# HaoZhongkai/DPOT

Measured on AMD Instinct MI355X. Metric: PDE samples/sec (128^2 x10 -> 1 rollout step), DPOT-Tiny train step, higher is better.
Workload: dtype f32

## Files before the change

### dpot_amd/_lib.py

```python
from __future__ import annotations

import ctypes as C
import os
import threading

HERE = os.path.dirname(os.path.abspath(__file__))
LIB_PATH = os.environ.get("DPOT_HIP_LIB") or os.path.join(HERE, "lib", "libdpot_hip.so")

c_fp = C.c_void_p
c_i = C.c_int
c_i64 = C.c_int64
c_f = C.c_float
c_d = C.c_double


class GemmDesc(C.Structure):
    _fields_ = [
        ("A", c_fp), ("B", c_fp), ("C", c_fp),
        ("M", C.c_int32), ("N", C.c_int32), ("K", C.c_int32),
        ("batch", C.c_int32),
        ("transA", C.c_int32), ("transB", C.c_int32),
        ("lda", C.c_int32), ("ldb", C.c_int32), ("ldc", C.c_int32),
        ("strideA", c_i64), ("strideB", c_i64), ("strideC", c_i64),
        ("bias", c_fp), ("strideBias", c_i64),
# ... 157 lines not shown
    "dpot_mlp_wgrad2": (c_i, [c_fp] * 4 + [c_i] * 3 + [c_fp] * 5 + [c_i, c_fp]),
    "dpot_afno_wgrad2_splitk": (c_i, [c_i] * 3),
    "dpot_afno_wgrad2_ws_elems": (c_i64, [c_i] * 3),
    "dpot_afno_wgrad2": (c_i, [c_fp] * 4 + [c_i] * 4 + [c_fp] * 5 + [c_i, c_fp]),
    "dpot_block_finalize": (c_i, [c_fp, c_i, c_i, c_i] + [c_fp] * 4 + [c_fp, c_i, c_i, c_i] + [c_fp] * 4 + [c_fp] * 3
                            + [c_i, c_i, c_i] + [c_fp] * 4 + [c_i, c_fp]),
    "dpot_bf16_pack_both_supported": (c_i, [c_i, c_i]),
    "dpot_bf16_pack_both": (c_i, [c_fp, c_i, c_i, c_i, c_fp, c_fp, c_fp, c_fp]),
    "dpot_bf16_pack_both_norm": (c_i, [c_fp, c_i, c_i, c_i, c_fp, c_fp, c_fp, c_fp, c_i, c_i, c_fp, c_fp, c_fp]),
    "dpot_embed_supported": (c_i, [c_i] * 5),
    "dpot_embed_wfrag_elems": (c_i, []),
    "dpot_embed_pack_w0": (c_i, [c_fp, c_i, c_fp, c_fp]),
    "dpot_embed_fwd": (c_i, [c_fp] * 5 + [c_i] * 6 + [c_fp]),
    "dpot_embed_wgrad_ws_elems": (c_i, [c_i] * 3),
    "dpot_embed_wgrad": (c_i, [c_fp] * 4 + [c_i] * 7 + [c_fp]),
    "dpot_gemm_panel_supported": (c_i, [c_i, c_i, c_i]),
    "dpot_gemm_panel": (c_i, [c_fp, c_i, c_fp, c_fp, c_fp, c_i, c_fp, c_i, c_fp, c_i, c_fp, c_i] + [c_i] * 5 + [c_fp]),
}

_lib = None
_lock = threading.Lock()


class DpotHipError(RuntimeError):
    pass


def lib_path() -> str:
    return LIB_PATH

# ... 26 lines not shown
```

### dpot_amd/build.py

```python
from __future__ import annotations

import os
import shutil
import subprocess
import sys
from concurrent.futures import ThreadPoolExecutor

HERE = os.path.dirname(os.path.abspath(__file__))
CSRC = os.path.join(HERE, "csrc")
LIBDIR = os.path.join(HERE, "lib")
LIB = os.path.join(LIBDIR, "libdpot_hip.so")
SOURCES = ["core.hip", "gemm.hip", "gemm_panel.hip", "gemm_tn.hip", "gemm_bf16p.hip", "afno_mlp.hip", "afno_mlp6.hip", "afno_fused.hip", "dft.hip", "norm.hip", "gn_dft.hip", "misc.hip", "loss_opt.hip", "metrics.hip", "tail.hip", "data.hip", "embed.hip", "resize.hip", "evalmetrics.hip"]
FLAGS = ["--offload-arch=gfx950", "-O3", "-std=c++17", "-fPIC", "-Wall", "-Wno-unused-function",
         "-Wno-pass-failed"]
EXTRA_FLAGS = {"afno_mlp6.hip": ["-fno-slp-vectorize"]}


def _hipcc() -> str:
    for cand in (os.environ.get("HIPCC"), shutil.which("hipcc"), "/opt/rocm/bin/hipcc"):
        if cand and os.path.exists(cand):
            return cand
    raise RuntimeError("hipcc not found (need ROCm >= 7.0 to build the gfx950 kernels)")


def _stale(target: str, deps) -> bool:
    if not os.path.exists(target):
        return True
    t = os.path.getmtime(target)
    return any(os.path.getmtime(d) > t for d in deps)


def build(force: bool = False, verbose: bool = True) -> str:
    hipcc = _hipcc()
    os.makedirs(LIBDIR, exist_ok=True)
    hdrs = [os.path.join(CSRC, "common.h"), os.path.join(CSRC, "dft_fast.h"), os.path.join(CSRC, "gemm_split.h"), os.path.join(CSRC, "gemm_epi.h"), os.path.join(CSRC, "gemm_bf16p_common.h"), os.path.join(os.path.dirname(HERE), "include", "dpot_hip.h")]
    objs, jobs = [], []
    for src in SOURCES:
        s = os.path.join(CSRC, src)
        o = os.path.join(LIBDIR, src.replace(".hip", ".o"))
        objs.append(o)
        if force or _stale(o, [s] + hdrs):
            jobs.append([hipcc] + FLAGS + EXTRA_FLAGS.get(src, []) + ["-c", s, "-o", o])

    def run(cmd):
        if verbose:
            print("[dpot_amd.build]", " ".join(cmd), flush=True)
        r = subprocess.run(cmd, capture_output=True, text=True)
        if r.returncode != 0:
            raise RuntimeError(f"hipcc failed:\n{' '.join(cmd)}\n{r.stdout}\n{r.stderr}")
        return r
# ... 12 lines not shown
```

### dpot_amd/csrc/embed.hip

```cpp
#include "common.h"

namespace dpot {

typedef float f32x4 __attribute__((ext_vector_type(4)));

constexpr int EM_P = 8;
constexpr int EM_C = 4;
constexpr int EM_NP = 4;
constexpr int EM_CT = 3;
constexpr int EM_LW = 2;
constexpr int EM_TMAX = 10;
constexpr int EM_KD = EM_C * EM_P * EM_P;
constexpr int EM_WFL = EM_P * 2 * EM_CT * 256;
constexpr int EM_GFL = EM_P * EM_NP * EM_P * EM_TMAX * EM_C;

struct EmbedArgs {
  const float* x;
  const float* wf;
  const float* bt;
  const float* dh;
  float* hpre;
  float* hh;
  float* part;
  int X, Y, T, h, w, hidp, act, ngroups, wq;
};

__device__ __forceinline__ void em_glds16(const float* g, float* l) {
  __builtin_amdgcn_global_load_lds((const __attribute__((address_space(1))) void*)g,
// ... 230 lines not shown
  for (int s = s0; s < s1; ++s) v += part[((long long)s * 48 + n) * EM_KD + k];
  red[sl][o] = v;
  __syncthreads();
  if (sl == 0 && ok) {
    float t = 0.f;
#pragma unroll
    for (int q = 0; q < 16; ++q) t += red[q][o];
    dw0[(long long)n * ldw + k] = t;
  }
}

__global__ __launch_bounds__(256) void embed_pack_w0_kernel(const float* __restrict__ w0, int hid, int K0,
                                                            float* __restrict__ wf) {
  const int idx = blockIdx.x * 256 + threadIdx.x;
  if (idx >= EM_WFL) return;
  const int jj = idx & 3, lane = (idx >> 2) & 63, blk = idx >> 8;
  const int ct = blk % EM_CT, ij = blk / EM_CT;
  const int jq = ij & 1, i = ij >> 1;
  const int n = ct * 16 + (lane & 15), c = lane >> 4;
  wf[idx] = n < hid ? w0[(long long)n * K0 + c * 64 + i * 8 + 4 * jq + jj] : 0.f;
}

}

using namespace dpot;

static int embed_grid(int ngroups) {
  int g = ngroups < 256 ? ngroups : 256;
  return g < 1 ? 1 : g;
}

extern "C" int dpot_embed_supported(int C, int P, int T, int hid, int w) {
  return C == EM_C && P == EM_P && T >= 1 && T <= EM_TMAX && hid >= 1 && hid <= 16 * EM_CT && w % EM_NP == 0;
}

// ... 62 lines not shown
```

### dpot_amd/functional.py

```python
from __future__ import annotations

import os
from collections import OrderedDict
from typing import Optional

import torch

from . import ops
from .ops import EPI_ACT, EPI_DACT

Tensor = torch.Tensor


def _pad4(n: int) -> int:
    return (n + 3) // 4 * 4


class _Sink:
    __slots__ = ("fp", "i")

    def __init__(self, param: Optional[Tensor], needed: bool):
        s = getattr(param, "_dpot_grad_slot", None) if (needed and param is not None) else None
        self.fp, self.i = s if s is not None else (None, -1)
        if self.fp is not None:
# ... 62 lines not shown

def embed_derived(pos, w0, b0, w2, b2, taw, tagamma, tt, T: int, grid=None, layouts=None):
    hid, E = w0.shape[0], w2.shape[0]
    K0 = w0[0].numel()
    hidp = _pad4(hid)
    tok = pos.shape[2] * pos.shape[3]
    dev = pos.device
    if layouts is not None:
        w0p, b0p, w2p, posb = layouts[0].view(hidp, K0), layouts[1].view(hidp), layouts[2].view(E, hidp), layouts[3].view(tok, E)
    else:
        w0p = ops.copy2d_pad(w0, hid, K0, hidp, K0)
        b0p = ops.copy2d_pad(b0, 1, hid, 1, hidp).view(hidp)
        w2p = ops.copy2d_pad(w2, E, hid, E, hidp)
        posT = ops.transpose2d(pos, 1, E, tok).view(tok, E)
        posb = ops.bias_add(posT, b2)
    ws = ops.timeagg_scale_w(taw, tagamma, tt) if tagamma is not None else taw
    V = torch.empty(T * hidp, E, dtype=torch.float32, device=dev)
    ops.gemm(w2p, ws, V, hidp, E, E, transA=True, lda=hidp, ldb=E, ldc=E, batch=T, strideA=0, strideB=E * E,
             strideC=hidp * E)
    wsum = ops.colsum(ws, T, E * E).view(E, E)
    cc = torch.empty(tok, E, dtype=torch.float32, device=dev)
    ops.gemm(posb, wsum, cc, tok, E, E, lda=E, ldb=E, ldc=E)
    wfrag = bt = None
    if grid is not None:
        kg = grid.shape[1]
        wfrag = ops.embed_pack_w0(w0)
        bt = torch.empty(grid.shape[0], hidp, dtype=torch.float32, device=dev)
        ops.gemm(grid, w0p[:, K0 - kg:], bt, grid.shape[0], hidp, kg, transB=True, lda=kg, ldb=K0, ldc=hidp, bias=b0p)
    return w0p, b0p, w2p, posb, ws, V, wsum, cc, wfrag, bt, grid

# ... 38 lines not shown
        _check_epoch(ctx, "EmbedFn")
        A0, Hpre, Hh, w0p, w2p, ws, V, wsum, posb, taw, tagamma, tt, grid = ctx.saved_tensors
        B, X, Y, T, Cc, P, h, w, hid, hidp, E, K0, act = ctx.dims
        s_pos, s_w0, s_b0, s_w2, s_b2, s_taw, s_gamma = ctx.sinks
        tok = h * w
        M, M0 = B * tok, B * tok * T
        dev = dY.device
        dY = dY.contiguous().view(M, E)
        dHpre = torch.empty(M0, hidp, dtype=torch.float32, device=dev)
        ops.gemm(dY, V, dHpre, M, T * hidp, E, transB=True, lda=E, ldb=E, ldc=T * hidp, act=act, mode=EPI_DACT,
                 aux=Hpre, ldaux=T * hidp)
        dV = torch.empty(T * hidp, E, dtype=torch.float32, device=dev)
        ops.gemm(Hh, dY, dV, T * hidp, E, M, transA=True, lda=T * hidp, ldb=E, ldc=E,
                 splitk=ops.auto_splitk(T * hidp, E, M, tn=True))
        dc = ops.group_rowsum(dY, B, tok, 1, E)
        dwsum = torch.empty(E, E, dtype=torch.float32, device=dev)
        ops.gemm(posb, dc, dwsum, E, E, tok, transA=True, lda=E, ldb=E, ldc=E, splitk=ops.auto_splitk(E, E, tok, tn=True))
        dposb = torch.empty(tok, E, dtype=torch.float32, device=dev)
        ops.gemm(dc, wsum, dposb, tok, E, E, transB=True, lda=E, ldb=E, ldc=E)
        dpos = s_pos.done(ops.transpose2d(dposb, 1, tok, E, out=s_pos.out()).view(1, E, h, w))
        db2 = s_b2.done(ops.colsum(dposb, tok, E, out=s_b2.out()))
        dw2_t = torch.empty(T, E, hidp, dtype=torch.float32, device=dev)
        ops.gemm(ws, dV, dw2_t, E, hidp, E, transB=True, lda=E, ldb=E, ldc=hidp, batch=T, strideA=E * E,
                 strideB=hidp * E, strideC=E * hidp)
        dw2p = ops.colsum(dw2_t, T, E * hidp).view(E, hidp)
        dw2 = s_w2.done(ops.copy2d_pad(dw2p, E, hidp, E, hid, out=s_w2.out()).view(E, hid, 1, 1))
        dws = s_taw.out() if tagamma is None else None
        dws = ops._out(dws, (T, E, E), dev)
        ops.gemm(w2p, dV, dws, E, E, hidp, lda=hidp, ldb=E, ldc=E, batch=T, strideA=0, strideB=hidp * E,
                 strideC=E * E, res=dwsum, ldres=E, strideRes=0)
        if tagamma is not None:
            dtaw, dgamma = ops.timeagg_scale_w_bwd(dws, taw, tagamma, tt, out_dw=s_taw.out(),
                                                   out_dgamma=s_gamma.out())
            dtaw, dgamma = s_taw.done(dtaw), s_gamma.done(dgamma)
        else:
            dtaw, dgamma = s_taw.done(dws), None
        if ctx.implicit:
            db0 = s_b0.done(ops.colsum(dHpre, M0, hid, ld=hidp, out=s_b0.out()))
            dw0 = ops._out(s_w0.out(), (hid, K0), dev)
            ops.embed_wgrad(A0, dHpre, dw0, hid)
            dHs = ops.group_rowsum(dHpre, B, tok * T, 1, hidp)
            kg = grid.shape[1]
            ops.gemm(dHs, grid, dw0[:, K0 - kg:], hid, kg, tok * T, transA=True, lda=hidp, ldb=kg, ldc=K0)
            dw0 = s_w0.done(dw0.view(hid, Cc + 3, P, P))
        elif hid == hidp:
            dw0p, db0 = ops.linear_bwd_wb(dHpre, A0, None, s_b0.out())
            db0 = s_b0.done(db0)
        else:
            db0 = s_b0.done(ops.colsum(dHpre, M0, hid, ld=hidp, out=s_b0.out()))
            dw0p = ops.linear_bwd_weight(dHpre, A0)
        if not ctx.implicit:
            dw0 = s_w0.done(ops.copy2d_pad(dw0p, hidp, K0, hid, K0, out=s_w0.out()).view(hid, Cc + 3, P, P))
        dx = None
        if ctx.needs_input_grad[0]:
            dA0 = ops.linear_bwd_data(dHpre, w0p)
            dx = ops.unpatchify(dA0, B, X, Y, T, Cc, P)
        return dx, dpos, dw0, db0, dw2, db2, dtaw, dgamma, None, None, None, None, None, None, None

# ... 651 lines not shown
```

### dpot_amd/ops.py

```python
from __future__ import annotations

import ctypes as C
import contextlib
import functools
import threading
import os
from typing import Optional, Tuple

import torch

from . import _lib
from ._lib import GemmDesc, check

Tensor = torch.Tensor

ACT_IDS = {None: 0, "none": 0, "gelu": 1, "tanh": 2, "sigmoid": 3, "relu": 4, "leaky_relu": 5, "softplus": 6,
           "ELU": 7, "silu": 8}
EPI_LINEAR, EPI_ACT, EPI_DACT, EPI_AFNO_WGRAD = 0, 1, 2, 3
GEMM_F32, GEMM_BF16X6, GEMM_AUTO, GEMM_BF16 = 0, 1, 2, 3
_PRECISIONS = {"f32": GEMM_F32, "bf16x6": GEMM_BF16X6, "auto": GEMM_AUTO, "bf16": GEMM_BF16}
_gemm_precision = _PRECISIONS[os.environ.get("DPOT_GEMM_PRECISION", "f32")]


def set_gemm_precision(name: str) -> None:
# ... 91 lines not shown
TUNE_KEYS = {
    "mixer": (3, "AFNO mixer MLP: 3 = three-product fused kernel (afno_mlp3), 4 = four-product fused kernel (afno_mlp2), "
                 "0 = two generic GEMM launches"),
    "afno_layer": (-1, "one-launch AFNO layer forward (afno_fused_fwd): -1 = where it measured faster (>= 80 % full last "
                       "round of (sample, block) workgroups), 0 = never, 1 = wherever supported"),
    "gn_fuse": (1, "0 = GroupNorm as its own kernels: not fused with the mixer's DFTs, never applied on the load of its consumer"),
    "panel": (1, "0 = generic GEMM kernels instead of the pre-packed-weight panel GEMM, the token-contraction weight-gradient "
                 "kernels (gemm_tn) and their two-layer launches"),
    "wgrad_gauss": (1, "0 = four-product AFNO weight gradients instead of the three-product forms"),
    "bf16p_bd": (1, "0 = the LDS-DMA bf16 GEMM kernels of rounds 2-3 for every launch instead of the B-direct kernels"),
    "bf16p_shape": (1, "0 = none of the bf16 GEMM shape heuristics: 128 x 256 tiles only, column-major tile order, eight waves, "
                       "un-paired weight gradients"),
    "packs": (1, "0 = bf16 packs by separate pack passes only: none from the one-launch AFNO layer, the GroupNorm backward or Adam"),
    "pack_both": (1, "0 = bf16 channel MLP without the pack-both path (one pack pass per operand form, fp32 pre-activation saved)"),
    "fused_small": (1, "0 = separate small launches: per-block reduce launches, eight layout launches, torch ops for the cls head"),
    "embed_implicit": (1, "0 = explicit patch matrix + GEMM instead of the implicit-GEMM patch embedding"),
    "mixer6": (1, "bf16x6 mixer kernel afno_mlp6 under gemm_precision 'auto' / 'bf16x6': 1 = where it measured faster (96 channels "
                  "per block: DPOT-L), 2 = wherever supported (also 128), 0 = never (the fp32 matrix-core kernels)"),
}


def _parse_tune():
    out = {}
    for kv in os.environ.get("DPOT_TUNE", "").split(","):
        kv = kv.strip()
        if not kv:
            continue
        k, _, v = kv.partition("=")
        if k not in TUNE_KEYS:
            raise ValueError(f"DPOT_TUNE: unknown key {k!r} (known: {', '.join(TUNE_KEYS)})")
        out[k] = int(v)
# ... 765 lines not shown
    M0 = B * (X // 8) * (Y // 8) * T
    hpre = torch.empty(M0, hidp, dtype=torch.float32, device=x.device)
    hh = torch.empty_like(hpre)
    check(_lib.load().dpot_embed_fwd(x.data_ptr(), wfrag.data_ptr(), btab.data_ptr(), hpre.data_ptr(), hh.data_ptr(),
                                     B, X, Y, T, hidp, act, _stream()), "embed_fwd")
    return hh, hpre


def embed_wgrad(x: Tensor, dhpre: Tensor, dw0: Tensor, hid: int) -> Tensor:
    lib = _lib.load()
    B, X, Y, T, _ = x.shape
    ws = torch.empty(lib.dpot_embed_wgrad_ws_elems(B, X, Y), dtype=torch.float32, device=x.device)
    check(lib.dpot_embed_wgrad(x.data_ptr(), dhpre.data_ptr(), ws.data_ptr(), dw0.data_ptr(), dw0.stride(0), hid, B, X,
                               Y, T, dhpre.shape[1], _stream()), "embed_wgrad")
    return dw0


def unpatchify(dA: Tensor, B: int, X: int, Y: int, T: int, Cc: int, P: int) -> Tensor:
    dx = torch.empty(B, X, Y, T, Cc, dtype=torch.float32, device=dA.device)
    check(_lib.load().dpot_unpatchify(dA.data_ptr(), dx.data_ptr(), B, X, Y, T, Cc, P, _stream()), "unpatchify")
    return dx


def pixel_shuffle(z: Tensor, B: int, h: int, w: int, P: int, Cc: int, inverse: bool = False) -> Tensor:
    out = torch.empty(B * h * w * P * P, Cc, dtype=torch.float32, device=z.device)
    if not inverse:
        out = out.view(B, h * P, w * P, Cc)
        check(_lib.load().dpot_pixel_shuffle(z.data_ptr(), out.data_ptr(), B, h, w, P, Cc, 0, _stream()),
              "pixel_shuffle")
    else:
# ... 729 lines not shown
```

### include/dpot_hip.h

```cpp
#ifndef DPOT_HIP_H
#define DPOT_HIP_H

#include <stdint.h>

#ifdef __cplusplus
extern "C" {
#endif

#define DPOT_OK 0
#define DPOT_EINVAL (-1)
#define DPOT_EUNSUP (-2)
#define DPOT_EHIP (-3)

typedef void* dpot_stream_t;

enum {
  DPOT_ACT_NONE = 0,
  DPOT_ACT_GELU = 1,
  DPOT_ACT_TANH = 2,
  DPOT_ACT_SIGMOID = 3,
  DPOT_ACT_RELU = 4,
  DPOT_ACT_LEAKY_RELU = 5,
  DPOT_ACT_SOFTPLUS = 6,
  DPOT_ACT_ELU = 7,
// ... 130 lines not shown
                        dpot_stream_t stream);

int dpot_patchify(const float* x, const float* gx, const float* gy, const float* gt, float* A, int B, int X,
                  int Y, int T, int C, int P, dpot_stream_t stream);
int dpot_unpatchify(const float* dA, float* dx, int B, int X, int Y, int T, int C, int P,
                    dpot_stream_t stream);

int dpot_embed_supported(int C, int P, int T, int hid, int w);
int dpot_embed_wfrag_elems(void);
int dpot_embed_pack_w0(const float* w0, int hid, float* wfrag, dpot_stream_t stream);
int dpot_embed_fwd(const float* x, const float* wfrag, const float* btab, float* hpre, float* hh, int B, int X, int Y,
                   int T, int hidp, int act, dpot_stream_t stream);
int dpot_embed_wgrad_ws_elems(int B, int X, int Y);
int dpot_embed_wgrad(const float* x, const float* dhpre, float* workspace, float* dw0, int ldw, int hid, int B, int X,
                     int Y, int T, int hidp, dpot_stream_t stream);
int dpot_pixel_shuffle(const float* z, float* out, int B, int h, int w, int P, int Cc, int inverse,
                       dpot_stream_t stream);
int dpot_copy2d_pad(const float* src, int sR, int sC, float* dst, int dR, int dC, dpot_stream_t stream);
int dpot_transpose2d(const float* src, float* dst, int nbatch, int R, int C, dpot_stream_t stream);
int dpot_colsum_parts(int M);
int dpot_colsum(const float* X, int M, int N, int ld, float* out, float* part, dpot_stream_t stream);
int dpot_colsum_scatter(const float* X, int M, int N, int ld, float* part, int nseg, const int* seg_start,
                        const int* seg_len, float* const* seg_dst, dpot_stream_t stream);
int dpot_group_rowsum(const float* X, float* out, int B, int R, int T, int N, dpot_stream_t stream);
int dpot_token_mean(const float* x, float* y, int B, int T, int E, dpot_stream_t stream);
int dpot_token_mean_bwd(const float* dy, const float* add, float* dx, int B, int T, int E,
                        dpot_stream_t stream);
int dpot_small_linear_supported(int M, int N, int K);
int dpot_small_linear(const float* x, int ldx, const float* W, int ldw, const float* bias, float* y, float* pre, int ldy,
                      int M, int N, int K, int act, dpot_stream_t stream);
// ... 177 lines not shown
```

Baseline: 10640.

## Fuse embed-fold weight-only algebra into multi-segment forward and backward kernels

Adds embed_fold kernels that compute the weight-only parts of the patch-embedding fold in a few segmented launches: the time-aggregation products V, the weight sum over T, the positional term, the grid bias table and the w0 fragment packing on the forward side, and dpos, db2, dw2, dtaw, dgamma and the grid part of dw0 on the backward side. These replace many separate generic GEMM, colsum and copy launches. The goal is to cut launch count and host overhead for small weight-only work on each train step. The cost is a large new code path with hand-written fp32 MFMA tiles and partial-sum workspaces that need their own reductions. It is gated by embed_implicit and E<=512.

After: 10630. Within noise of the previous version (-0.1%).

```diff
diff --git a/dpot_amd/_lib.py b/dpot_amd/_lib.py
--- a/dpot_amd/_lib.py
+++ b/dpot_amd/_lib.py
@@ -195,6 +195,10 @@
     "dpot_embed_fwd": (c_i, [c_fp] * 5 + [c_i] * 6 + [c_fp]),
     "dpot_embed_wgrad_ws_elems": (c_i, [c_i] * 3),
     "dpot_embed_wgrad": (c_i, [c_fp] * 4 + [c_i] * 7 + [c_fp]),
+    "dpot_embed_fold_supported": (c_i, [c_i] * 4),
+    "dpot_embed_fold_bwd_ws_elems": (c_i64, [c_i] * 5),
+    "dpot_embed_fold_fwd": (c_i, [c_fp] * 15 + [c_i] * 7 + [c_fp]),
+    "dpot_embed_fold_bwd": (c_i, [c_fp] * 16 + [c_i, c_fp] + [c_i] * 7 + [c_fp]),
     "dpot_gemm_panel_supported": (c_i, [c_i, c_i, c_i]),
     "dpot_gemm_panel": (c_i, [c_fp, c_i, c_fp, c_fp, c_fp, c_i, c_fp, c_i, c_fp, c_i, c_fp, c_i] + [c_i] * 5 + [c_fp]),
 }
diff --git a/dpot_amd/build.py b/dpot_amd/build.py
--- a/dpot_amd/build.py
+++ b/dpot_amd/build.py
@@ -10,7 +10,7 @@
 CSRC = os.path.join(HERE, "csrc")
 LIBDIR = os.path.join(HERE, "lib")
 LIB = os.path.join(LIBDIR, "libdpot_hip.so")
-SOURCES = ["core.hip", "gemm.hip", "gemm_panel.hip", "gemm_tn.hip", "gemm_bf16p.hip", "afno_mlp.hip", "afno_mlp6.hip", "afno_fused.hip", "dft.hip", "norm.hip", "gn_dft.hip", "misc.hip", "loss_opt.hip", "metrics.hip", "tail.hip", "data.hip", "embed.hip", "resize.hip", "evalmetrics.hip"]
+SOURCES = ["core.hip", "gemm.hip", "gemm_panel.hip", "gemm_tn.hip", "gemm_bf16p.hip", "afno_mlp.hip", "afno_mlp6.hip", "afno_fused.hip", "dft.hip", "norm.hip", "gn_dft.hip", "misc.hip", "loss_opt.hip", "metrics.hip", "tail.hip", "data.hip", "embed.hip", "embed_fold.hip", "resize.hip", "evalmetrics.hip"]
 FLAGS = ["--offload-arch=gfx950", "-O3", "-std=c++17", "-fPIC", "-Wall", "-Wno-unused-function",
          "-Wno-pass-failed"]
 EXTRA_FLAGS = {"afno_mlp6.hip": ["-fno-slp-vectorize"]}
@@ -33,7 +33,7 @@
 def build(force: bool = False, verbose: bool = True) -> str:
     hipcc = _hipcc()
     os.makedirs(LIBDIR, exist_ok=True)
-    hdrs = [os.path.join(CSRC, "common.h"), os.path.join(CSRC, "dft_fast.h"), os.path.join(CSRC, "gemm_split.h"), os.path.join(CSRC, "gemm_epi.h"), os.path.join(CSRC, "gemm_bf16p_common.h"), os.path.join(os.path.dirname(HERE), "include", "dpot_hip.h")]
+    hdrs = [os.path.join(CSRC, "common.h"), os.path.join(CSRC, "dft_fast.h"), os.path.join(CSRC, "gemm_split.h"), os.path.join(CSRC, "gemm_epi.h"), os.path.join(CSRC, "gemm_bf16p_common.h"), os.path.join(CSRC, "embed_pack.h"), os.path.join(os.path.dirname(HERE), "include", "dpot_hip.h")]
     objs, jobs = [], []
     for src in SOURCES:
         s = os.path.join(CSRC, src)
diff --git a/dpot_amd/csrc/embed.hip b/dpot_amd/csrc/embed.hip
--- a/dpot_amd/csrc/embed.hip
+++ b/dpot_amd/csrc/embed.hip
@@ -1,17 +1,12 @@
 #include "common.h"
+#include "embed_pack.h"
 
 namespace dpot {
 
 typedef float f32x4 __attribute__((ext_vector_type(4)));
 
-constexpr int EM_P = 8;
-constexpr int EM_C = 4;
-constexpr int EM_NP = 4;
-constexpr int EM_CT = 3;
 constexpr int EM_LW = 2;
 constexpr int EM_TMAX = 10;
-constexpr int EM_KD = EM_C * EM_P * EM_P;
-constexpr int EM_WFL = EM_P * 2 * EM_CT * 256;
 constexpr int EM_GFL = EM_P * EM_NP * EM_P * EM_TMAX * EM_C;
 
 struct EmbedArgs {
@@ -272,11 +267,7 @@
                                                             float* __restrict__ wf) {
   const int idx = blockIdx.x * 256 + threadIdx.x;
   if (idx >= EM_WFL) return;
-  const int jj = idx & 3, lane = (idx >> 2) & 63, blk = idx >> 8;
-  const int ct = blk % EM_CT, ij = blk / EM_CT;
-  const int jq = ij & 1, i = ij >> 1;
-  const int n = ct * 16 + (lane & 15), c = lane >> 4;
-  wf[idx] = n < hid ? w0[(long long)n * K0 + c * 64 + i * 8 + 4 * jq + jj] : 0.f;
+  wf[idx] = em_pack_w0_elem(w0, hid, K0, idx);
 }
 
 }
diff --git a/dpot_amd/csrc/embed_fold.hip b/dpot_amd/csrc/embed_fold.hip
--- /dev/null
+++ b/dpot_amd/csrc/embed_fold.hip
@@ -0,0 +1,440 @@
+#include "common.h"
+#include "embed_pack.h"
+
+namespace dpot {
+
+typedef float ef_f32x4 __attribute__((ext_vector_type(4)));
+
+constexpr int EF_KC = 32;
+constexpr int EF_LD = 65;
+constexpr int EF_EMAX = 2048;
+constexpr int EF_TMAX = 64;
+constexpr int EF_WR = 4;
+constexpr int EF_KS = 256;
+
+struct EfArgs {
+  const float *taw, *gamma, *tt, *w2p, *posb, *w0, *w0p, *b0p, *grid, *wsum_in, *dV, *dc, *dHs;
+  float *V, *wsum, *cc, *wfrag, *bt, *ws, *dpos, *db2, *dw2, *dtaw, *dgamma, *dw0;
+  float *k_dwsum, *k_db2, *k_dw2, *k_dw0, *k_dg;
+  int T, E, hidp, hid, tok, K0, kg, R, ldw0;
+  int e0, e1, e2, e3;
+  int nks, nrt, njt;
+};
+
+__device__ __forceinline__ float ef_cos(const EfArgs& a, int t, int i) {
+  return a.gamma ? cosf(a.tt[t] * a.gamma[i]) : 1.f;
+}
+
+template <int BM, int BN, bool AKF, bool BKF, class FA, class FB>
+__device__ __forceinline__ void ef_gemm(ef_f32x4 (&acc)[BM / 32][BN / 32], int K, FA fa, FB fb, float* As, float* Bs) {
+  constexpr int NA = BM * EF_KC / 256, NB = BN * EF_KC / 256, TM = BM / 32, TN = BN / 32;
+  const int tid = threadIdx.x, lane = tid & 63, wid = tid >> 6;
+  const int wm = (wid & 1) * (BM / 2), wn = (wid >> 1) * (BN / 2);
+  float ra[NA], rb[NB];
+#pragma unroll
+  for (int i = 0; i < TM; ++i)
+#pragma unroll
+    for (int j = 0; j < TN; ++j) acc[i][j] = ef_f32x4{0.f, 0.f, 0.f, 0.f};
+  auto gload = [&](int k0) {
+#pragma unroll
+    for (int r = 0; r < NA; ++r) {
+      const int idx = tid + 256 * r;
+      const int k = AKF ? idx % EF_KC : idx / BM, m = AKF ? idx / EF_KC : idx % BM;
+      ra[r] = k0 + k < K ? fa(m, k0 + k) : 0.f;
+    }
+#pragma unroll
+    for (int r = 0; r < NB; ++r) {
+      const int idx = tid + 256 * r;
+      const int k = BKF ? idx % EF_KC : idx / BN, n = BKF ? idx / EF_KC : idx % BN;
+      rb[r] = k0 + k < K ? fb(k0 + k, n) : 0.f;
+    }
+  };
+  gload(0);
+  for (int k0 = 0; k0 < K; k0 += EF_KC) {
+#pragma unroll
+    for (int r = 0; r < NA; ++r) {
+      const int idx = tid + 256 * r;
+      const int k = AKF ? idx % EF_KC : idx / BM, m = AKF ? idx / EF_KC : idx % BM;
+      As[k * EF_LD + m] = ra[r];
+    }
+#pragma unroll
+    for (int r = 0; r < NB; ++r) {
+      const int idx = tid + 256 * r;
+      const int k = BKF ? idx % EF_KC : idx / BN, n = BKF ? idx / EF_KC : idx % BN;
+      Bs[k * EF_LD + n] = rb[r];
+    }
+    __syncthreads();
+    if (k0 + EF_KC < K) gload(k0 + EF_KC);
+    const int kend = min(EF_KC, K - k0);
+    for (int kk = 0; kk < kend; kk += 4) {
+      const int kr = (kk + (lane >> 4)) * EF_LD + (lane & 15);
+      float af[TM], bf[TN];
+#pragma unroll
+      for (int i = 0; i < TM; ++i) af[i] = As[kr + wm + i * 16];
+#pragma unroll
+      for (int j = 0; j < TN; ++j) bf[j] = Bs[kr + wn + j * 16];
+#pragma unroll
+      for (int i = 0; i < TM; ++i)
+#pragma unroll
+        for (int j = 0; j < TN; ++j) acc[i][j] = __builtin_amdgcn_mfma_f32_16x16x4f32(af[i], bf[j], acc[i][j], 0, 0, 0);
+    }
+    __syncthreads();
+  }
+}
+
+template <int BM, int BN, class EPI>
+__device__ __forceinline__ void ef_epilogue(const ef_f32x4 (&acc)[BM / 32][BN / 32], EPI epi) {
+  const int lane = threadIdx.x & 63, wid = threadIdx.x >> 6;
+  const int wm = (wid & 1) * (BM / 2), wn = (wid >> 1) * (BN / 2);
+#pragma unroll
+  for (int i = 0; i < BM / 32; ++i)
+#pragma unroll
+    for (int j = 0; j < BN / 32; ++j)
+#pragma unroll
+      for (int r = 0; r < 4; ++r) epi(wm + i * 16 + 4 * (lane >> 4) + r, wn + j * 16 + (lane & 15), acc[i][j][r]);
+}
+
+template <int BM, int BN, class F>
+__device__ __forceinline__ float ef_rowsum(const ef_f32x4 (&acc)[BM / 32][BN / 32], F f, float* red) {
+  const int lane = threadIdx.x & 63, wid = threadIdx.x >> 6;
+  const int wm = (wid & 1) * (BM / 2), wn = (wid >> 1) * (BN / 2);
+#pragma unroll
+  for (int i = 0; i < BM / 32; ++i)
+#pragma unroll
+    for (int r = 0; r < 4; ++r) {
+      const int m = wm + i * 16 + 4 * (lane >> 4) + r;
+      float s = 0.f;
+#pragma unroll
+      for (int j = 0; j < BN / 32; ++j) s += f(m, wn + j * 16 + (lane & 15), acc[i][j][r]);
+#pragma unroll
+      for (int off = 8; off > 0; off >>= 1) s += __shfl_xor(s, off, 64);
+      if ((lane & 15) == 0) red[(wid >> 1) * BM + m] = s;
+    }
+  __syncthreads();
+  return threadIdx.x < BM ? red[threadIdx.x] + red[BM + threadIdx.x] : 0.f;
+}
+
+__global__ __launch_bounds__(256) void embed_fold_fwd_kernel(const EfArgs a) {
+  __shared__ float As[EF_KC * EF_LD], Bs[EF_KC * EF_LD], aux[EF_EMAX];
+  const int tid = threadIdx.x, E = a.E, hidp = a.hidp;
+  int b = blockIdx.x;
+  if (b < a.e0) {
+    const int nct = E / 32, t = b / nct, j0 = (b - t * nct) * 32;
+    for (int i = tid; i < E; i += 256) aux[i] = ef_cos(a, t, i);
+    __syncthreads();
+    const float* tw = a.taw + (long long)t * E * E;
+    ef_f32x4 acc[2][1];
+    ef_gemm<64, 32, false, false>(
+        acc, E, [&](int m, int k) { return m < hidp ? a.w2p[k * hidp + m] : 0.f; },
+        [&](int k, int n) { return tw[(long long)k * E + j0 + n] * aux[k]; }, As, Bs);
+    float* Vt = a.V + (long long)t * hidp * E;
+    ef_epilogue<64, 32>(acc, [&](int m, int n, float v) {
+      if (m < hidp) Vt[(long long)m * E + j0 + n] = v;
+    });
+    return;
+  }
+  b -= a.e0;
+  if (b < a.e1 - a.e0) {
+    const int i0 = b * EF_WR, T = a.T;
+    for (int q = tid; q < T * EF_WR; q += 256) aux[q] = ef_cos(a, q / EF_WR, min(i0 + q % EF_WR, E - 1));
+    __syncthreads();
+    for (int e = tid; e < EF_WR * E; e += 256) {
+      const int r = e / E, j = e - r * E, i = i0 + r;
+      if (i >= E) break;
+      float s = 0.f;
+      for (int t = 0; t < T; ++t) {
+        const long long o = ((long long)t * E + i) * E + j;
+        const float v = a.taw[o] * aux[t * EF_WR + r];
+        if (a.ws) a.ws[o] = v;
+        s += v;
+      }
+      a.wsum[(long long)i * E + j] = s;
+    }
+    return;
+  }
+  b -= a.e1 - a.e0;
+  if (b < a.e2 - a.e1) {
+    const int q0 = b * 64, kg = a.kg, R = a.R, K0 = a.K0;
+    ef_f32x4 acc[2][2];
+    ef_gemm<64, 64, true, true>(
+        acc, kg, [&](int m, int k) { return q0 + m < R ? a.grid[(long long)(q0 + m) * kg + k] : 0.f; },
+        [&](int k, int n) { return n < hidp ? a.w0p[(long long)n * K0 + (K0 - kg) + k] : 0.f; }, As, Bs);
+    ef_epilogue<64, 64>(acc, [&](int m, int n, float v) {
+      if (q0 + m < R && n < hidp) a.bt[(long long)(q0 + m) * hidp + n] = v + a.b0p[n];
+    });
+    return;
+  }
+  b -= a.e2 - a.e1;
+  const int idx = b * 256 + tid;
+  if (idx < EM_WFL) a.wfrag[idx] = em_pack_w0_elem(a.w0, a.hid, a.K0, idx);
+}
+
+template <int BT>
+__global__ __launch_bounds__(256) void embed_fold_cc_kernel(const EfArgs a) {
+  __shared__ float As[EF_KC * EF_LD], Bs[EF_KC * EF_LD];
+  const int E = a.E, tok = a.tok, nct = E / BT;
+  const int r0 = (blockIdx.x / nct) * BT, j0 = (blockIdx.x % nct) * BT;
+  ef_f32x4 acc[BT / 32][BT / 32];
+  ef_gemm<BT, BT, true, false>(
+      acc, E, [&](int m, int k) { return r0 + m < tok ? a.posb[(long long)(r0 + m) * E + k] : 0.f; },
+      [&](int k, int n) { return a.wsum[(long long)k * E + j0 + n]; }, As, Bs);
+  ef_epilogue<BT, BT>(acc, [&](int m, int n, float v) {
+    if (r0 + m < tok) a.cc[(long long)(r0 + m) * E + j0 + n] = v;
+  });
+}
+
+template <int BT>
+__global__ __launch_bounds__(256) void embed_fold_bwd1_kernel(const EfArgs a) {
+  __shared__ float As[EF_KC * EF_LD], Bs[EF_KC * EF_LD], aux[128];
+  const int tid = threadIdx.x, E = a.E, hidp = a.hidp, tok = a.tok;
+  int b = blockIdx.x;
+  if (b < a.e0) {
+    const int nrt = (tok + BT - 1) / BT, it = b / nrt, rt = b - it * nrt;
+    const int i0 = it * BT, r0 = rt * BT;
+    ef_f32x4 acc[BT / 32][BT / 32];
+    ef_gemm<BT, BT, true, true>(
+        acc, E, [&](int m, int k) { return a.wsum_in[(long long)(i0 + m) * E + k]; },
+        [&](int k, int n) { return r0 + n < tok ? a.dc[(long long)(r0 + n) * E + k] : 0.f; }, As, Bs);
+    ef_epilogue<BT, BT>(acc, [&](int m, int n, float v) {
+      if (r0 + n < tok) a.dpos[(long long)(i0 + m) * tok + r0 + n] = v;
+    });
+    const float s = ef_rowsum<BT, BT>(acc, [&](int, int n, float v) { return r0 + n < tok ? v : 0.f; }, aux);
+    if (tid < BT) a.k_db2[(long long)rt * E + i0 + tid] = s;
+    return;
+  }
+  b -= a.e0;
+  if (b < a.e1 - a.e0) {
+    const int nct = E / BT, i0 = (b / nct) * BT, j0 = (b % nct) * BT;
+    ef_f32x4 acc[BT / 32][BT / 32];
+    ef_gemm<BT, BT, false, false>(
+        acc, tok, [&](int m, int k) { return a.posb[(long long)k * E + i0 + m]; },
+        [&](int k, int n) { return a.dc[(long long)k * E + j0 + n]; }, As, Bs);
+    ef_epilogue<BT, BT>(acc, [&](int m, int n, float v) { a.k_dwsum[(long long)(i0 + m) * E + j0 + n] = v; });
+    return;
+  }
+  b -= a.e1 - a.e0;
+  if (b < a.e2 - a.e1) {
+    const int nit = E / 32, t = b / nit, i0 = (b - t * nit) * 32;
+    if (tid < 32) aux[tid] = ef_cos(a, t, i0 + tid);
+    __syncthreads();
+    const float* tw = a.taw + (long long)t * E * E;
+    const float* dVt = a.dV + (long long)t * hidp * E;
+    ef_f32x4 acc[1][2];
+    ef_gemm<32, 64, true, true>(
+        acc, E, [&](int m, int k) { return tw[(long long)(i0 + m) * E + k] * aux[m]; },
+        [&](int k, int n) { return n < hidp ? dVt[(long long)n * E + k] : 0.f; }, As, Bs);
+    float* part = a.k_dw2 + (long long)t * E * hidp;
+    ef_epilogue<32, 64>(acc, [&](int m, int n, float v) {
+      if (n < hidp) part[(long long)(i0 + m) * hidp + n] = v;
+    });
+    return;
+  }
+  b -= a.e2 - a.e1;
+  {
+    const int kg = a.kg, R = a.R, nkt = (kg + 31) / 32;
+    const int s = b / nkt, c0 = (b - s * nkt) * 32;
+    const int q0 = s * EF_KS, kl = min(EF_KS, R - q0);
+    ef_f32x4 acc[2][1];
+    ef_gemm<64, 32, false, false>(
+        acc, kl, [&](int m, int k) { return m < hidp ? a.dHs[(long long)(q0 + k) * hidp + m] : 0.f; },
+        [&](int k, int n) { return c0 + n < kg ? a.grid[(long long)(q0 + k) * kg + c0 + n] : 0.f; }, As, Bs);
+    float* part = a.k_dw0 + (long long)s * hidp * kg;
+    ef_epilogue<64, 32>(acc, [&](int m, int n, float v) {
+      if (m < hidp && c0 + n < kg) part[(long long)m * kg + c0 + n] = v;
+    });
+  }
+}
+
+__global__ __launch_bounds__(256) void embed_fold_bwd2_kernel(const EfArgs a) {
+  __shared__ float As[EF_KC * EF_LD], Bs[EF_KC * EF_LD], aux[128], red[128];
+  const int tid = threadIdx.x, E = a.E, hidp = a.hidp, T = a.T;
+  int b = blockIdx.x;
+  if (b < a.e0) {
+    const int nt = E / 64, t = b / (nt * nt), q = b - t * nt * nt, i0 = (q / nt) * 64, jt = q % nt, j0 = jt * 64;
+    if (tid < 64) {
+      float cs = 1.f, coef = 0.f;
+      if (a.gamma) {
+        const float tv = a.tt[t], arg = tv * a.gamma[i0 + tid];
+        cs = cosf(arg);
+        coef = -sinf(arg) * tv;
+      }
+      aux[tid] = cs;
+      aux[64 + tid] = coef;
+    }
+    __syncthreads();
+    const float* dVt = a.dV + (long long)t * hidp * E;
+    ef_f32x4 acc[2][2];
+    ef_gemm<64, 64, true, false>(
+        acc, hidp, [&](int m, int k) { return a.w2p[(long long)(i0 + m) * hidp + k]; },
+        [&](int k, int n) { return dVt[(long long)k * E + j0 + n]; }, As, Bs);
+    const long long base = (long long)t * E * E;
+#pragma unroll
+    for (int i = 0; i < 2; ++i)
+#pragma unroll
+      for (int j = 0; j < 2; ++j)
+#pragma unroll
+        for (int r = 0; r < 4; ++r) {
+          const int lane = tid & 63, wid = tid >> 6;
+          const int m = (wid & 1) * 32 + i * 16 + 4 * (lane >> 4) + r, n = (wid >> 1) * 32 + j * 16 + (lane & 15);
+          acc[i][j][r] += a.k_dwsum[(long long)(i0 + m) * E + j0 + n];
+        }
+    ef_epilogue<64, 64>(acc, [&](int m, int n, float v) {
+      a.dtaw[base + (long long)(i0 + m) * E + j0 + n] = v * aux[m];
+    });
+    if (a.gamma) {
+      const float s = ef_rowsum<64, 64>(
+          acc, [&](int m, int n, float v) { return v * a.taw[base + (long long)(i0 + m) * E + j0 + n]; }, red);
+      if (tid < 64) a.k_dg[((long long)t * a.njt + jt) * E + i0 + tid] = s * aux[64 + tid];
+    }
+    return;
+  }
+  b -= a.e0;
+  if (b < a.e1 - a.e0) {
+    const int i = b * 256 + tid;
+    if (i < E) {
+      float s = 0.f;
+      for (int p = 0; p < a.nrt; ++p) s += a.k_db2[(long long)p * E + i];
+      a.db2[i] = s;
+    }
+    return;
+  }
+  b -= a.e1 - a.e0;
+  if (b < a.e2 - a.e1) {
+    const int idx = b * 256 + tid, hid = a.hid;
+    if (idx < E * hid) {
+      const int i = idx / hid, h = idx - i * hid;
+      float s = 0.f;
+      for (int t = 0; t < T; ++t) s += a.k_dw2[((long long)t * E + i) * hidp + h];
+      a.dw2[idx] = s;
+    }
+    return;
+  }
+  b -= a.e2 - a.e1;
+  {
+    const int idx = b * 256 + tid, kg = a.kg, nks = a.nks;
+    if (idx < a.hid * kg) {
+      const int n = idx / kg, k = idx - n * kg;
+      float s = 0.f;
+      for (int p = 0; p < nks; ++p) s += a.k_dw0[((long long)p * hidp + n) * kg + k];
+      a.dw0[(long long)n * a.ldw0 + (a.K0 - kg) + k] = s;
+    }
+  }
+}
+
+__global__ __launch_bounds__(256) void embed_fold_dgamma_kernel(const float* __restrict__ part, int nparts, int E,
+                                                                float* __restrict__ dgamma) {
+  const int i = blockIdx.x * 256 + threadIdx.x;
+  if (i >= E) return;
+  float s = 0.f;
+  for (int p = 0; p < nparts; ++p) s += part[(long long)p * E + i];
+  dgamma[i] = s;
+}
+
+}
+
+using namespace dpot;
+
+static int ef_tile(int E, int tok) { return (long long)((tok + 63) / 64) * (E / 64) >= 256 ? 64 : 32; }
+
+extern "C" int dpot_embed_fold_supported(int T, int E, int hidp, int tok) {
+  return T >= 1 && T <= EF_TMAX && E >= 64 && E <= EF_EMAX && E % 64 == 0 && hidp >= 4 && hidp <= 64 && hidp % 4 == 0 &&
+         tok >= 1 && tok <= 65536;
+}
+
+struct EfLayout {
+  int bt, nrt, nks;
+  long long o_dwsum, o_db2, o_dw2, o_dw0, o_dg, total;
+};
+static EfLayout ef_layout(int T, int E, int hidp, int tok, int kg) {
+  EfLayout l;
+  l.bt = ef_tile(E, tok);
+  l.nrt = (tok + l.bt - 1) / l.bt;
+  l.nks = kg > 0 ? (tok * T + EF_KS - 1) / EF_KS : 0;
+  l.o_dwsum = 0;
+  l.o_db2 = l.o_dwsum + (long long)E * E;
+  l.o_dw2 = l.o_db2 + (long long)l.nrt * E;
+  l.o_dw0 = l.o_dw2 + (long long)T * E * hidp;
+  l.o_dg = l.o_dw0 + (long long)l.nks * hidp * kg;
+  l.total = l.o_dg + (long long)T * (E / 64) * E;
+  return l;
+}
+
+extern "C" long long dpot_embed_fold_bwd_ws_elems(int T, int E, int hidp, int tok, int kg) {
+  if (!dpot_embed_fold_supported(T, E, hidp, tok) || kg < 0) return 0;
+  return ef_layout(T, E, hidp, tok, kg).total;
+}
+
+extern "C" int dpot_embed_fold_fwd(const float* taw, const float* gamma, const float* tt, const float* w2p,
+                                   const float* posb, const float* w0, const float* w0p, const float* b0p,
+                                   const float* grid, float* V, float* wsum, float* cc, float* wfrag, float* bt,
+                                   float* ws, int T, int E, int hidp, int hid, int tok, int K0, int kg,
+                                   dpot_stream_t stream) {
+  DPOT_REQUIRE(dpot_embed_fold_supported(T, E, hidp, tok), "embed_fold_fwd: unsupported shape T=%d E=%d hidp=%d tok=%d", T,
+               E, hidp, tok);
+  DPOT_REQUIRE(taw && tt && w2p && posb && V && wsum && cc && hid >= 1 && hid <= hidp, "embed_fold_fwd: bad argument");
+  DPOT_REQUIRE(!grid || (w0 && w0p && b0p && wfrag && bt && kg >= 1 && kg <= K0 && hid <= 16 * EM_CT &&
+                         K0 == (EM_C + 3) * EM_P * EM_P),
+               "embed_fold_fwd: bad grid-part argument");
+  EfArgs a{};
+  a.taw = taw; a.gamma = gamma; a.tt = tt; a.w2p = w2p; a.posb = posb; a.w0 = w0; a.w0p = w0p; a.b0p = b0p; a.grid = grid;
+  a.V = V; a.wsum = wsum; a.cc = cc; a.wfrag = wfrag; a.bt = bt; a.ws = ws;
+  a.T = T; a.E = E; a.hidp = hidp; a.hid = hid; a.tok = tok; a.K0 = K0; a.kg = grid ? kg : 0; a.R = tok * T;
+  a.e0 = T * (E / 32);
+  a.e1 = a.e0 + (E + EF_WR - 1) / EF_WR;
+  a.e2 = a.e1 + (grid ? (a.R + 63) / 64 : 0);
+  a.e3 = a.e2 + (grid ? EM_WFL / 256 : 0);
+  hipLaunchKernelGGL(embed_fold_fwd_kernel, dim3(a.e3), dim3(256), 0, as_stream(stream), a);
+  int rc = check_launch("embed_fold_fwd_kernel");
+  if (rc) return rc;
+  const int bt_ = ef_tile(E, tok);
+  const int nblk = ((tok + bt_ - 1) / bt_) * (E / bt_);
+  if (bt_ == 64)
+    hipLaunchKernelGGL(embed_fold_cc_kernel<64>, dim3(nblk), dim3(256), 0, as_stream(stream), a);
+  else
+    hipLaunchKernelGGL(embed_fold_cc_kernel<32>, dim3(nblk), dim3(256), 0, as_stream(stream), a);
+  return check_launch("embed_fold_cc_kernel");
+}
+
+extern "C" int dpot_embed_fold_bwd(const float* dV, const float* dc, const float* dHs, const float* taw,
+                                   const float* gamma, const float* tt, const float* w2p, const float* posb,
+                                   const float* wsum, const float* grid, float* dpos, float* db2, float* dw2, float* dtaw,
+                                   float* dgamma, float* dw0, int ldw0, float* workspace, int T, int E, int hidp, int hid,
+                                   int tok, int K0, int kg, dpot_stream_t stream) {
+  DPOT_REQUIRE(dpot_embed_fold_supported(T, E, hidp, tok), "embed_fold_bwd: unsupported shape T=%d E=%d hidp=%d tok=%d", T,
+               E, hidp, tok);
+  DPOT_REQUIRE(dV && dc && taw && tt && w2p && posb && wsum && dpos && db2 && dw2 && dtaw && workspace && hid >= 1 &&
+                   hid <= hidp && (!gamma || dgamma),
+               "embed_fold_bwd: bad argument");
+  DPOT_REQUIRE(!grid || (dHs && dw0 && kg >= 1 && kg <= K0 && ldw0 >= K0), "embed_fold_bwd: bad grid-part argument");
+  if (!grid) kg = 0;
+  const EfLayout l = ef_layout(T, E, hidp, tok, kg);
+  EfArgs a{};
+  a.dV = dV; a.dc = dc; a.dHs = dHs; a.taw = taw; a.gamma = gamma; a.tt = tt; a.w2p = w2p; a.posb = posb;
+  a.wsum_in = wsum; a.grid = grid;
+  a.dpos = dpos; a.db2 = db2; a.dw2 = dw2; a.dtaw = dtaw; a.dgamma = dgamma; a.dw0 = dw0; a.ldw0 = ldw0;
+  a.k_dwsum = workspace + l.o_dwsum; a.k_db2 = workspace + l.o_db2; a.k_dw2 = workspace + l.o_dw2;
+  a.k_dw0 = workspace + l.o_dw0; a.k_dg = workspace + l.o_dg;
+  a.T = T; a.E = E; a.hidp = hidp; a.hid = hid; a.tok = tok; a.K0 = K0; a.kg = kg; a.R = tok * T;
+  a.nks = l.nks; a.nrt = l.nrt;
+  a.njt = E / 64;
+  a.e0 = (E / l.bt) * l.nrt;
+  a.e1 = a.e0 + (E / l.bt) * (E / l.bt);
+  a.e2 = a.e1 + T * (E / 32);
+  a.e3 = a.e2 + l.nks * ((kg + 31) / 32);
+  if (l.bt == 64)
+    hipLaunchKernelGGL(embed_fold_bwd1_kernel<64>, dim3(a.e3), dim3(256), 0, as_stream(stream), a);
+  else
+    hipLaunchKernelGGL(embed_fold_bwd1_kernel<32>, dim3(a.e3), dim3(256), 0, as_stream(stream), a);
+  int rc = check_launch("embed_fold_bwd1_kernel");
+  if (rc) return rc;
+  a.e0 = T * (E / 64) * (E / 64);
+  a.e1 = a.e0 + (E + 255) / 256;
+  a.e2 = a.e1 + (E * hid + 255) / 256;
+  a.e3 = a.e2 + (hid * kg + 255) / 256;
+  hipLaunchKernelGGL(embed_fold_bwd2_kernel, dim3(a.e3), dim3(256), 0, as_stream(stream), a);
+  rc = check_launch("embed_fold_bwd2_kernel");
+  if (rc || !gamma) return rc;
+  hipLaunchKernelGGL(embed_fold_dgamma_kernel, dim3((E + 255) / 256), dim3(256), 0, as_stream(stream),
+                     (const float*)a.k_dg, T * a.njt, E, dgamma);
+  return check_launch("embed_fold_dgamma_kernel");
+}
diff --git a/dpot_amd/csrc/embed_pack.h b/dpot_amd/csrc/embed_pack.h
--- /dev/null
+++ b/dpot_amd/csrc/embed_pack.h
@@ -0,0 +1,20 @@
+#pragma once
+
+namespace dpot {
+
+constexpr int EM_P = 8;
+constexpr int EM_C = 4;
+constexpr int EM_NP = 4;
+constexpr int EM_CT = 3;
+constexpr int EM_KD = EM_C * EM_P * EM_P;
+constexpr int EM_WFL = EM_P * 2 * EM_CT * 256;
+
+__device__ __forceinline__ float em_pack_w0_elem(const float* __restrict__ w0, int hid, int K0, int idx) {
+  const int jj = idx & 3, lane = (idx >> 2) & 63, blk = idx >> 8;
+  const int ct = blk % EM_CT, ij = blk / EM_CT;
+  const int jq = ij & 1, i = ij >> 1;
+  const int n = ct * 16 + (lane & 15), c = lane >> 4;
+  return n < hid ? w0[(long long)n * K0 + c * 64 + i * 8 + 4 * jq + jj] : 0.f;
+}
+
+}
diff --git a/dpot_amd/functional.py b/dpot_amd/functional.py
--- a/dpot_amd/functional.py
+++ b/dpot_amd/functional.py
@@ -100,6 +100,11 @@
         w2p = ops.copy2d_pad(w2, E, hid, E, hidp)
         posT = ops.transpose2d(pos, 1, E, tok).view(tok, E)
         posb = ops.bias_add(posT, b2)
+    if ops.embed_fold_supported(T, E, hidp, tok):
+        g = grid is not None
+        V, wsum, cc, wfrag, bt, ws = ops.embed_fold_fwd(taw, tagamma, tt, w2p, posb, hid, w0 if g else None,
+                                                        w0p if g else None, b0p if g else None, grid)
+        return w0p, b0p, w2p, posb, ws, V, wsum, cc, wfrag, bt, grid
     ws = ops.timeagg_scale_w(taw, tagamma, tt) if tagamma is not None else taw
     V = torch.empty(T * hidp, E, dtype=torch.float32, device=dev)
     ops.gemm(w2p, ws, V, hidp, E, E, transA=True, lda=hidp, ldb=E, ldc=E, batch=T, strideA=0, strideB=E * E,
@@ -168,6 +173,8 @@
         ops.gemm(Hh, dY, dV, T * hidp, E, M, transA=True, lda=T * hidp, ldb=E, ldc=E,
                  splitk=ops.auto_splitk(T * hidp, E, M, tn=True))
         dc = ops.group_rowsum(dY, B, tok, 1, E)
+        if ws is None:
+            return EmbedFn._backward_fold(ctx, dHpre, dV, dc)
         dwsum = torch.empty(E, E, dtype=torch.float32, device=dev)
         ops.gemm(posb, dc, dwsum, E, E, tok, transA=True, lda=E, ldb=E, ldc=E, splitk=ops.auto_splitk(E, E, tok, tn=True))
         dposb = torch.empty(tok, E, dtype=torch.float32, device=dev)
@@ -196,6 +203,46 @@
             dHs = ops.group_rowsum(dHpre, B, tok * T, 1, hidp)
             kg = grid.shape[1]
             ops.gemm(dHs, grid, dw0[:, K0 - kg:], hid, kg, tok * T, transA=True, lda=hidp, ldb=kg, ldc=K0)
+            dw0 = s_w0.done(dw0.view(hid, Cc + 3, P, P))
+        elif hid == hidp:
+            dw0p, db0 = ops.linear_bwd_wb(dHpre, A0, None, s_b0.out())
+            db0 = s_b0.done(db0)
+        else:
+            db0 = s_b0.done(ops.colsum(dHpre, M0, hid, ld=hidp, out=s_b0.out()))
+            dw0p = ops.linear_bwd_weight(dHpre, A0)
+        if not ctx.implicit:
+            dw0 = s_w0.done(ops.copy2d_pad(dw0p, hidp, K0, hid, K0, out=s_w0.out()).view(hid, Cc + 3, P, P))
+        dx = None
+        if ctx.needs_input_grad[0]:
+            dA0 = ops.linear_bwd_data(dHpre, w0p)
+            dx = ops.unpatchify(dA0, B, X, Y, T, Cc, P)
+        return dx, dpos, dw0, db0, dw2, db2, dtaw, dgamma, None, None, None, None, None, None, None
+
+    @staticmethod
+    def _backward_fold(ctx, dHpre, dV, dc):
+        A0, Hpre, Hh, w0p, w2p, ws, V, wsum, posb, taw, tagamma, tt, grid = ctx.saved_tensors
+        B, X, Y, T, Cc, P, h, w, hid, hidp, E, K0, act = ctx.dims
+        s_pos, s_w0, s_b0, s_w2, s_b2, s_taw, s_gamma = ctx.sinks
+        tok = h * w
+        M0 = B * tok * T
+        dev = dHpre.device
+        dHs = dw0 = None
+        if ctx.implicit:
+            dHs = ops.group_rowsum(dHpre, B, tok * T, 1, hidp)
+            dw0 = ops._out(s_w0.out(), (hid, K0), dev)
+        dpos, db2, dw2, dtaw, dgamma = ops.embed_fold_bwd(
+            dV, dc, taw, tagamma, tt, w2p, posb, wsum, hid, dHs=dHs, grid=grid if ctx.implicit else None, dw0=dw0,
+            out_dpos=s_pos.out(), out_db2=s_b2.out(), out_dw2=s_w2.out(), out_dtaw=s_taw.out(),
+            out_dgamma=s_gamma.out() if tagamma is not None else None)
+        dpos = s_pos.done(dpos.view(1, E, h, w))
+        db2 = s_b2.done(db2)
+        dw2 = s_w2.done(dw2.view(E, hid, 1, 1))
+        dtaw = s_taw.done(dtaw)
+        if tagamma is not None:
+            dgamma = s_gamma.done(dgamma)
+        if ctx.implicit:
+            db0 = s_b0.done(ops.colsum(dHpre, M0, hid, ld=hidp, out=s_b0.out()))
+            ops.embed_wgrad(A0, dHpre, dw0, hid)
             dw0 = s_w0.done(dw0.view(hid, Cc + 3, P, P))
         elif hid == hidp:
             dw0p, db0 = ops.linear_bwd_wb(dHpre, A0, None, s_b0.out())
diff --git a/dpot_amd/ops.py b/dpot_amd/ops.py
--- a/dpot_amd/ops.py
+++ b/dpot_amd/ops.py
@@ -129,7 +129,8 @@
     "packs": (1, "0 = bf16 packs by separate pack passes only: none from the one-launch AFNO layer, the GroupNorm backward or Adam"),
     "pack_both": (1, "0 = bf16 channel MLP without the pack-both path (one pack pass per operand form, fp32 pre-activation saved)"),
     "fused_small": (1, "0 = separate small launches: per-block reduce launches, eight layout launches, torch ops for the cls head"),
-    "embed_implicit": (1, "0 = explicit patch matrix + GEMM instead of the implicit-GEMM patch embedding"),
+    "embed_implicit": (1, "0 = explicit patch matrix + GEMM instead of the implicit-GEMM patch embedding, and the embed fold's "
+                          "weight-only algebra as generic GEMM / colsum / copy launches instead of embed_fold"),
     "mixer6": (1, "bf16x6 mixer kernel afno_mlp6 under gemm_precision 'auto' / 'bf16x6': 1 = where it measured faster (96 channels "
                   "per block: DPOT-L), 2 = wherever supported (also 128), 0 = never (the fp32 matrix-core kernels)"),
 }
@@ -925,6 +926,59 @@
     check(lib.dpot_embed_wgrad(x.data_ptr(), dhpre.data_ptr(), ws.data_ptr(), dw0.data_ptr(), dw0.stride(0), hid, B, X,
                                Y, T, dhpre.shape[1], _stream()), "embed_wgrad")
     return dw0
+
+
+EMBED_FOLD_MAX_E = 512
+
+
+def embed_fold_supported(T: int, E: int, hidp: int, tok: int) -> bool:
+    return (tune("embed_implicit") != 0 and E <= EMBED_FOLD_MAX_E
+            and bool(_lib.load().dpot_embed_fold_supported(T, E, hidp, tok)))
+
+
+def embed_fold_fwd(taw: Tensor, gamma: Optional[Tensor], tt: Tensor, w2p: Tensor, posb: Tensor, hid: int,
+                   w0: Optional[Tensor] = None, w0p: Optional[Tensor] = None, b0p: Optional[Tensor] = None,
+                   grid: Optional[Tensor] = None, want_ws: bool = False):
+    lib = _lib.load()
+    T, E, _ = taw.shape
+    hidp, tok, dev = w2p.shape[1], posb.shape[0], taw.device
+    V = torch.empty(T * hidp, E, dtype=torch.float32, device=dev)
+    wsum = torch.empty(E, E, dtype=torch.float32, device=dev)
+    cc = torch.empty(tok, E, dtype=torch.float32, device=dev)
+    ws = torch.empty(T, E, E, dtype=torch.float32, device=dev) if want_ws else None
+    wfrag = bt = None
+    K0 = kg = 0
+    if grid is not None:
+        K0, kg = w0p.shape[1], grid.shape[1]
+        wfrag = torch.empty(lib.dpot_embed_wfrag_elems(), dtype=torch.float32, device=dev)
+        bt = torch.empty(grid.shape[0], hidp, dtype=torch.float32, device=dev)
+    check(lib.dpot_embed_fold_fwd(taw.data_ptr(), _p(gamma), tt.data_ptr(), w2p.data_ptr(), posb.data_ptr(), _p(w0), _p(w0p),
+                                  _p(b0p), _p(grid), V.data_ptr(), wsum.data_ptr(), cc.data_ptr(), _p(wfrag), _p(bt), _p(ws),
+                                  T, E, hidp, hid, tok, K0, kg, _stream()), "embed_fold_fwd")
+    return V, wsum, cc, wfrag, bt, ws
+
+
+def embed_fold_bwd(dV: Tensor, dc: Tensor, taw: Tensor, gamma: Optional[Tensor], tt: Tensor, w2p: Tensor, posb: Tensor,
+                   wsum: Tensor, hid: int, dHs: Optional[Tensor] = None, grid: Optional[Tensor] = None,
+                   dw0: Optional[Tensor] = None, out_dpos: Optional[Tensor] = None, out_db2: Optional[Tensor] = None,
+                   out_dw2: Optional[Tensor] = None, out_dtaw: Optional[Tensor] = None, out_dgamma: Optional[Tensor] = None):
+    lib = _lib.load()
+    T, E, _ = taw.shape
+    hidp, tok, dev = w2p.shape[1], posb.shape[0], taw.device
+    K0 = kg = ldw0 = 0
+    if grid is not None:
+        K0, kg, ldw0 = dw0.shape[1], grid.shape[1], dw0.stride(0)
+    dpos = _out(out_dpos, (E, tok), dev)
+    db2 = _out(out_db2, (E,), dev)
+    dw2 = _out(out_dw2, (E, hid), dev)
+    dtaw = _out(out_dtaw, (T, E, E), dev)
+    dgamma = _out(out_dgamma, (1, E), dev) if gamma is not None else None
+    wk = torch.empty(lib.dpot_embed_fold_bwd_ws_elems(T, E, hidp, tok, kg), dtype=torch.float32, device=dev)
+    check(lib.dpot_embed_fold_bwd(dV.data_ptr(), dc.data_ptr(), _p(dHs), taw.data_ptr(), _p(gamma), tt.data_ptr(),
+                                  w2p.data_ptr(), posb.data_ptr(), wsum.data_ptr(), _p(grid), dpos.data_ptr(), db2.data_ptr(),
+                                  dw2.data_ptr(), dtaw.data_ptr(), _p(dgamma), _p(dw0), ldw0, wk.data_ptr(), T, E, hidp, hid,
+                                  tok, K0, kg, _stream()), "embed_fold_bwd")
+    return dpos, db2, dw2, dtaw, dgamma
 
 
 def unpatchify(dA: Tensor, B: int, X: int, Y: int, T: int, Cc: int, P: int) -> Tensor:
diff --git a/include/dpot_hip.h b/include/dpot_hip.h
--- a/include/dpot_hip.h
+++ b/include/dpot_hip.h
@@ -168,6 +168,16 @@
 int dpot_embed_wgrad_ws_elems(int B, int X, int Y);
 int dpot_embed_wgrad(const float* x, const float* dhpre, float* workspace, float* dw0, int ldw, int hid, int B, int X,
                      int Y, int T, int hidp, dpot_stream_t stream);
+int dpot_embed_fold_supported(int T, int E, int hidp, int tok);
+long long dpot_embed_fold_bwd_ws_elems(int T, int E, int hidp, int tok, int kg);
+int dpot_embed_fold_fwd(const float* taw, const float* gamma, const float* tt, const float* w2p, const float* posb,
+                        const float* w0, const float* w0p, const float* b0p, const float* grid, float* V, float* wsum,
+                        float* cc, float* wfrag, float* bt, float* ws, int T, int E, int hidp, int hid, int tok, int K0,
+                        int kg, dpot_stream_t stream);
+int dpot_embed_fold_bwd(const float* dV, const float* dc, const float* dHs, const float* taw, const float* gamma,
+                        const float* tt, const float* w2p, const float* posb, const float* wsum, const float* grid,
+                        float* dpos, float* db2, float* dw2, float* dtaw, float* dgamma, float* dw0, int ldw0,
+                        float* workspace, int T, int E, int hidp, int hid, int tok, int K0, int kg, dpot_stream_t stream);
 int dpot_pixel_shuffle(const float* z, float* out, int B, int h, int w, int P, int Cc, int inverse,
                        dpot_stream_t stream);
 int dpot_copy2d_pad(const float* src, int sR, int sC, float* dst, int dR, int dC, dpot_stream_t stream);
```
